# cvg/glue-factory

Hardware: AMD Instinct MI355X
Metric: image-pairs/sec (train step) SP+LightGlue N=2048 d=256 L=9 (higher is better)
Workload: dtype bf16; 1 GPU; configs[1]: SuperPoint + LightGlue train step -- frozen SuperPoint-open forward on 2x32 synthetic 1024x1024 images resident in HBM (view1 = view0 warped by a sampled homography, SURVEY 8(d)(P); first block and the 64-channel 3x3 blocks as fused HIP kernels, library convolutions + fused HIP tails for the 128/256-channel blocks), homography ground truth (gf_gt_nn), LightGlue fwd + loss + bwd + fused; pairs_per_gpu=32, global_batch=32, keypoints=2048, descriptor_dim=256, layers=9, parallelism=dp1

## Files before the change

glue-factory_amd/csrc/assignment.hip:

```cpp
#include <cstdlib>
#include "gf_common.h"
#include "assign_common.h"
#include "gf_amd.h"

#ifndef GF_WRITE_SPLIT
#define GF_WRITE_SPLIT 4
#endif
#ifndef GF_WRITE_ABL
#define GF_WRITE_ABL 0
#endif
#ifndef GF_BWD_SPLIT
#define GF_BWD_SPLIT 4
#endif

namespace {
template <typename T, int D, bool HAS_BIAS>
__global__ __launch_bounds__(256) void rows_lse_kernel(HeadParams p) {
    GF_HEAD_PROLOGUE(T, D)
    float m = GF_NEG_BIG, lsum = 0.f;
    const float* sb = p.sbias ? p.sbias + (int64_t)b * p.Ns : nullptr;
    auto bias = [&](int si, float& v0, float& v1) {
        const float x = sb ? sb[min(si, p.Ns - 1)] * GF_LOG2E : 0.f;
        v0 = si < p.Ns ? x : -INFINITY;
        v1 = 0.f;
    };
    auto body = [&](const T* tile, const float* vec0, const float*, int s0) {
        f32x16 s[2];
        float mx = GF_NEG_BIG;
        const bool plain = !HAS_BIAS && s0 + 64 <= p.Ns;
#pragma unroll
        for (int kb = 0; kb < 2; ++kb) {
#pragma unroll
            for (int r = 0; r < 16; ++r) s[kb][r] = 0.f;
            mma_tile<T, D>(s[kb], tile, kb * 32, of, l31, hi);
            if (plain) {
#pragma unroll
                for (int r = 0; r < 16; ++r) mx = fmaxf(mx, s[kb][r]);
            } else {
#pragma unroll
                for (int g = 0; g < 4; ++g) {
                    f32x4 b4 = *reinterpret_cast<const f32x4*>(vec0 + kb * 32 + 8 * g + 4 * hi);
#pragma unroll
                    for (int e = 0; e < 4; ++e) {
                        float x = s[kb][4 * g + e] * GF_LOG2E + b4[e];
                        s[kb][4 * g + e] = x;
                        mx = fmaxf(mx, x);
                    }
                }
            }
        }
        if (plain) mx *= GF_LOG2E;
        mx = fmaxf(mx, xhalf(mx));
        const float mnew = fmaxf(m, mx);
        float ps = 0.f;
#pragma unroll
        for (int kb = 0; kb < 2; ++kb)
#pragma unroll
            for (int r = 0; r < 16; ++r)
                ps += plain ? fast_exp2(fmaf(s[kb][r], GF_LOG2E, -mnew)) : fast_exp2(s[kb][r] - mnew);
        lsum = lsum * fast_exp2(m - mnew) + ps;
        m = mnew;
    };
    stream_tiles<T, D>(tiles, vecs, othp, 0, p.Ns, p.Ns, bias, body);
    lsum += xhalf(lsum);
    if (orow < p.No && hi == 0) p.f0[(int64_t)b * p.No + orow] = (m + fast_log2(lsum)) * GF_LN2;
}

template <typename T, int D>
__global__ __launch_bounds__(256) void rows_argmax_kernel(HeadParams p) {
    GF_HEAD_PROLOGUE(T, D)
    float best = -INFINITY;
    int bidx = 0x7fffffff;
    const float* sb = p.sbias ? p.sbias + (int64_t)b * p.Ns : nullptr;
    auto bias = [&](int si, float& v0, float& v1) {
        const float x = sb ? sb[min(si, p.Ns - 1)] : 0.f;
        v0 = si < p.Ns ? x : -INFINITY;
        v1 = 0.f;
    };
    auto body = [&](const T* tile, const float* vec0, const float*, int s0) {
        TileArg ta;
        ta.reset();
#pragma unroll
        for (int kb = 0; kb < 2; ++kb) {
            f32x16 s;
#pragma unroll
            for (int r = 0; r < 16; ++r) s[r] = 0.f;
            mma_tile<T, D>(s, tile, kb * 32, of, l31, hi);
#pragma unroll
            for (int g = 0; g < 4; ++g) {
                f32x4 b4 = *reinterpret_cast<const f32x4*>(vec0 + kb * 32 + 8 * g + 4 * hi);
#pragma unroll
                for (int e = 0; e < 4; ++e) {
                    ta.see(p.alpha * s[4 * g + e] + b4[e], kb * 32 + 8 * g + e);
                }
            }
        }
        ta.merge(s0, hi, best, bidx);
    };
    stream_tiles<T, D>(tiles, vecs, othp, 0, p.Ns, p.Ns, bias, body);
    float ob_ = xhalf(best);
    int oi = __shfl_xor(bidx, 32);
    if (ob_ > best || (ob_ == best && oi < bidx)) { best = ob_; bidx = oi; }
    if (orow < p.No && hi == 0) {
        p.f0[(int64_t)b * p.No + orow] = best;
        p.i0[(int64_t)b * p.No + orow] = (bidx == 0x7fffffff) ? 0 : bidx;
    }
}

template <typename T, int D, bool WITH_LSE>
__global__ __launch_bounds__(256, sizeof(T) == 2 ? 2 : 1) void rows_lse_argmax_kernel(HeadParams p) {
    GF_HEAD_PROLOGUE(T, D)
    float m = GF_NEG_BIG, lsum = 0.f;
    float best = -INFINITY;
    int bidx = 0x7fffffff;
    const float* zb = p.g0 + (int64_t)b * p.Ns;
    const float* nb = p.g1 + (int64_t)b * p.Ns;
    auto bias = [&](int si, float& v0, float& v1) {
        const int sc = min(si, p.Ns - 1);
        const float z = zb[sc];
        const float x = fminf(z, 0.f) - log1pf(__expf(-fabsf(z))) - nb[sc];
        v0 = si < p.Ns ? x : -INFINITY;
        v1 = si < p.Ns ? 0.f : -INFINITY;
    };
    auto body = [&](const T* tile, const float* vec0, const float* vec1, int s0) {
        f32x16 s[2];
        float mx = GF_NEG_BIG;
        TileArg ta;
        ta.reset();
#pragma unroll
        for (int kb = 0; kb < 2; ++kb) {
#pragma unroll
            for (int r = 0; r < 16; ++r) s[kb][r] = 0.f;
            mma_tile<T, D>(s[kb], tile, kb * 32, of, l31, hi);
#pragma unroll
            for (int g = 0; g < 4; ++g) {
                f32x4 b4 = *reinterpret_cast<const f32x4*>(vec0 + kb * 32 + 8 * g + 4 * hi);
#pragma unroll
                for (int e = 0; e < 4; ++e) {
                    const float raw = s[kb][4 * g + e];
                    ta.see(p.alpha * raw + b4[e], kb * 32 + 8 * g + e);
                    if (WITH_LSE) mx = fmaxf(mx, raw);
                }
            }
        }
        ta.merge(s0, hi, best, bidx);
        if (WITH_LSE) {
            if (s0 + 64 > p.Ns) {
                mx = GF_NEG_BIG;
#pragma unroll
                for (int kb = 0; kb < 2; ++kb)
#pragma unroll
                    for (int g = 0; g < 4; ++g) {
                        f32x4 v4 = *reinterpret_cast<const f32x4*>(vec1 + kb * 32 + 8 * g + 4 * hi);
#pragma unroll
                        for (int e = 0; e < 4; ++e) {
                            s[kb][4 * g + e] += v4[e];
                            mx = fmaxf(mx, s[kb][4 * g + e]);
                        }
                    }
            }
            mx *= GF_LOG2E;
            mx = fmaxf(mx, xhalf(mx));
            const float mnew = fmaxf(m, mx);
            float ps = 0.f;
#pragma unroll
            for (int kb = 0; kb < 2; ++kb)
#pragma unroll
                for (int r = 0; r < 16; ++r) ps += fast_exp2(fmaf(s[kb][r], GF_LOG2E, -mnew));
            lsum = lsum * fast_exp2(m - mnew) + ps;
            m = mnew;
        }
    };
    stream_tiles<T, D>(tiles, vecs, othp, 0, p.Ns, p.Ns, bias, body);
    float ob_ = xhalf(best);
    int oi = __shfl_xor(bidx, 32);
    if (ob_ > best || (ob_ == best && oi < bidx)) { best = ob_; bidx = oi; }
    if (WITH_LSE) lsum += xhalf(lsum);
    if (orow < p.No && hi == 0) {
        p.f0[(int64_t)b * p.No + orow] = best;
        p.i0[(int64_t)b * p.No + orow] = (bidx == 0x7fffffff) ? 0 : bidx;
        if (WITH_LSE) p.f1[(int64_t)b * p.No + orow] = (m + fast_log2(lsum)) * GF_LN2;
    }
}

template <typename T, int D>
__global__ __launch_bounds__(256) void assign_write_kernel(HeadParams p) {
    GF_HEAD_PROLOGUE(T, D)
#ifdef GF_WRITE_LDPAD
    const int64_t ldo = (p.No + 1 + GF_WRITE_LDPAD - 1) / GF_WRITE_LDPAD * GF_WRITE_LDPAD;
    float* out = reinterpret_cast<float*>(p.out) + (int64_t)b * (p.Ns + 1) * ldo;
#else
    float* out = reinterpret_cast<float*>(p.out) + (int64_t)b * (p.Ns + 1) * (p.No + 1);
    const int64_t ldo = p.No + 1;
#endif
    const float ocb = p.obias ? p.obias[(int64_t)b * p.No + old_] : 0.f;
    const float* sb = p.sbias ? p.sbias + (int64_t)b * p.Ns : nullptr;
    auto bias = [&](int si, float& v0, float& v1) {
        v0 = sb ? sb[min(si, p.Ns - 1)] : 0.f;
        v1 = 0.f;
    };
    float esum = 0.f;
    auto body = [&](const T* tile, const float* vec0, const float*, int s0) {
        TileArg ta;
        ta.reset();
#pragma unroll
        for (int kb = 0; kb < 2; ++kb) {
            f32x16 s;
#pragma unroll
            for (int r = 0; r < 16; ++r) s[r] = 0.f;
            if (!(GF_WRITE_ABL & 1)) mma_tile<T, D>(s, tile, kb * 32, of, l31, hi);
#pragma unroll
            for (int g = 0; g < 4; ++g) {
                f32x4 b4 = *reinterpret_cast<const f32x4*>(vec0 + kb * 32 + 8 * g + 4 * hi);
#pragma unroll
                for (int e = 0; e < 4; ++e) {
                    int si = s0 + kb * 32 + 8 * g + 4 * hi + e;
                    if (si < p.Ns && orow < p.No) {
                        const float v = p.alpha * s[4 * g + e] + b4[e] + ocb;
                        if (!(GF_WRITE_ABL & 2)) out[(int64_t)si * ldo + orow] = v;
                        else if (v == 12345.678f) out[0] = v;
                        if (p.f0 && !(GF_WRITE_ABL & 4)) esum += fast_exp2(v * GF_LOG2E);
                    }
                }
            }
        }
    };
    const int per = ((p.Ns + 63) / 64 + nsp - 1) / nsp * 64;
    const int s_begin = split * per, s_end = min(p.Ns, s_begin + per);
    if (s_begin < s_end) stream_tiles<T, D>(tiles, vecs, othp, s_begin, s_end, p.Ns, bias, body);
    if (split == 0 && orow < p.No && hi == 0) out[(int64_t)p.Ns * ldo + orow] = p.g1 ? p.g1[(int64_t)b * p.No + orow] : 0.f;
    if (ob == 0 && split == 0) {
        for (int si = threadIdx.x; si < p.Ns; si += 256) {
            const float v = p.g0 ? p.g0[(int64_t)b * p.Ns + si] : 0.f;
            out[(int64_t)si * ldo + p.No] = v;
            if (p.f0) esum += fast_exp2(v * GF_LOG2E);
        }
        if (threadIdx.x == 0) out[(int64_t)p.Ns * ldo + p.No] = p.corner;
    }
    if (p.f0) {
        esum = wave_allsum(esum);
        if ((threadIdx.x & 63) == 0) atomicAdd(p.f0 + b, esum);
    }
}

template <typename T, int D>
__global__ __launch_bounds__(256) void dual_softmax_bwd_kernel(HeadParams p) {
    GF_HEAD_PROLOGUE(T, D)
    T* dS = reinterpret_cast<T*>(p.out) + (int64_t)b * p.Ns * p.No;
    const float c2 = p.g1[(int64_t)b * p.No + old_] * GF_LOG2E;
    const float gco = p.g3[(int64_t)b * p.No + old_];
    const float* Gb = p.G ? p.G + (int64_t)b * (p.Ns + 1) * p.ldg : nullptr;
    const int per = ((p.Ns + 63) / 64 + nsp - 1) / nsp * 64;
    const int s_begin = split * per, s_end = min(p.Ns, s_begin + per);
    const float* rb = p.g0 + (int64_t)b * p.Ns;
    const float* grb = p.g2 + (int64_t)b * p.Ns;
    auto bias = [&](int si, float& v0, float& v1) {
        const int sc = min(si, p.Ns - 1);
        const float r_ = rb[sc] * GF_LOG2E, g_ = grb[sc];
        v0 = si < p.Ns ? r_ : INFINITY;
        v1 = si < p.Ns ? g_ : 0.f;
    };
    auto body = [&](const T* tile, const float* vec0, const float* vec1, int s0) {
#pragma unroll
        for (int kb = 0; kb < 2; ++kb) {
            f32x16 s;
#pragma unroll
            for (int r = 0; r < 16; ++r) s[r] = 0.f;
            mma_tile<T, D>(s, tile, kb * 32, of, l31, hi);
#pragma unroll
            for (int g = 0; g < 4; ++g) {
                f32x4 r4 = *reinterpret_cast<const f32x4*>(vec0 + kb * 32 + 8 * g + 4 * hi);
                f32x4 g4 = *reinterpret_cast<const f32x4*>(vec1 + kb * 32 + 8 * g + 4 * hi);
#pragma unroll
                for (int e = 0; e < 4; ++e) {
                    int si = s0 + kb * 32 + 8 * g + 4 * hi + e;
                    if (si < p.Ns && orow < p.No) {
                        float x = s[4 * g + e] * GF_LOG2E;
                        float v = fast_exp2(x - r4[e]) * g4[e] + fast_exp2(x - c2) * gco;
                        if (Gb) v += p.galpha * Gb[(int64_t)si * p.ldg + orow];
                        dS[(int64_t)si * p.No + orow] = from_f32<T>(v);
                    }
                }
            }
        }
    };
    stream_tiles<T, D>(tiles, vecs, othp, s_begin, s_end, p.Ns, bias, body);
}

__global__ void filter_matches_kernel(const float* max0, const int64_t* arg0, const int64_t* arg1, float th,
                                      int64_t* m0, int64_t* m1, float* s0, float* s1, int B, int M, int N) {
    int64_t t = (int64_t)blockIdx.x * blockDim.x + threadIdx.x;
    int64_t tot = (int64_t)B * (M + N);
    if (t >= tot) return;
    int b = t / (M + N);
    int k = t % (M + N);
    const int64_t* a0 = arg0 + (int64_t)b * M;
    const int64_t* a1 = arg1 + (int64_t)b * N;
    if (k < M) {
        int64_t j = a0[k];
        bool mutual = (a1[j] == k);
        float sc = mutual ? __expf(max0[(int64_t)b * M + k]) : 0.f;
        s0[(int64_t)b * M + k] = sc;
        m0[(int64_t)b * M + k] = (mutual && sc > th) ? j : -1;
    } else {
        int j = k - M;
        int64_t i = a1[j];
        bool mutual = (a0[i] == j);
        float sc = mutual ? __expf(max0[(int64_t)b * M + i]) : 0.f;
        s1[(int64_t)b * N + j] = sc;
        m1[(int64_t)b * N + j] = (mutual && sc > th) ? i : -1;
    }
}

enum { K_LSE, K_ARGMAX, K_WRITE, K_BWD, K_LSEARG, K_ZNARG };

template <typename T, int D> int launch_td(int which, const HeadParams& p, hipStream_t st) {
    const int total = ((p.No + 127) / 128) * p.B * (p.nsplit > 1 ? p.nsplit : 1);
    const size_t lds = head_lds<T, D>();
#define GF_LAUNCH(kern)                                             \
    {                                                               \
        if (int e = set_lds(kern<T, D>, lds)) return e;             \
        kern<T, D><<<dim3(total), dim3(256), lds, st>>>(p);         \
        return (int)hipGetLastError();                              \
    }
    switch (which) {
        case K_LSE:
            if (p.sbias) {
                if (int e = set_lds(rows_lse_kernel<T, D, true>, lds)) return e;
                rows_lse_kernel<T, D, true><<<dim3(total), dim3(256), lds, st>>>(p);
            } else {
                if (int e = set_lds(rows_lse_kernel<T, D, false>, lds)) return e;
                rows_lse_kernel<T, D, false><<<dim3(total), dim3(256), lds, st>>>(p);
            }
            return (int)hipGetLastError();
        case K_ARGMAX: GF_LAUNCH(rows_argmax_kernel)
        case K_WRITE: GF_LAUNCH(assign_write_kernel)
        case K_BWD: GF_LAUNCH(dual_softmax_bwd_kernel)
        default: break;
    }
#undef GF_LAUNCH
#define GF_LAUNCH2(flag)                                                              \
    {                                                                                 \
        if (int e = set_lds(rows_lse_argmax_kernel<T, D, flag>, lds)) return e;       \
        rows_lse_argmax_kernel<T, D, flag><<<dim3(total), dim3(256), lds, st>>>(p);   \
        return (int)hipGetLastError();                                                \
    }
    if (which == K_LSEARG) GF_LAUNCH2(true)
    GF_LAUNCH2(false)
#undef GF_LAUNCH2
}

template <typename T> int launch_t(int which, const HeadParams& p, int D, hipStream_t st) {
    switch (D) {
        case 64: return launch_td<T, 64>(which, p, st);
        case 128: return launch_td<T, 128>(which, p, st);
        case 256: return launch_td<T, 256>(which, p, st);
        default: return GF_ERR_UNSUPPORTED;
    }
}

int rejected(const HeadParams& p, int D, int dtype) {
    if (p.B <= 0 || p.No <= 0 || p.Ns <= 0) return GF_ERR_SHAPE;
    if (dtype != GF_F32 && dtype != GF_BF16) return GF_ERR_DTYPE;
    if (D != 64 && D != 128 && D != 256) return GF_ERR_UNSUPPORTED;
    return 0;
}

int launch(int which, const HeadParams& p, int D, int dtype, void* stream) {
    if (p.B <= 0 || p.No <= 0 || p.Ns <= 0) return GF_ERR_SHAPE;
    hipStream_t st = reinterpret_cast<hipStream_t>(stream);
    if (dtype == GF_F32) return launch_t<float>(which, p, D, st);
    if (dtype == GF_BF16) return launch_t<bf16_t>(which, p, D, st);
    return GF_ERR_DTYPE;
}

}

extern "C" int gf_rows_lse(const void* a, const void* b, const float* colbias, float* lse,
                           int B, int M, int N, int D, int dtype, void* stream) {
    HeadParams p = {};
    p.own = a; p.oth = b; p.B = B; p.No = M; p.Ns = N; p.sbias = colbias; p.f0 = lse;
    return launch(K_LSE, p, D, dtype, stream);
}

extern "C" int gf_rows_argmax(const void* a, const void* b, const float* colbias, float alpha,
                              float* rowmax, int64_t* rowarg,
                              int B, int M, int N, int D, int dtype, void* stream) {
    HeadParams p = {};
    p.own = a; p.oth = b; p.B = B; p.No = M; p.Ns = N; p.sbias = colbias; p.alpha = alpha;
    p.f0 = rowmax; p.i0 = rowarg;
    return launch(K_ARGMAX, p, D, dtype, stream);
}

extern "C" int gf_rows_lse_argmax(const void* a, const void* b, const float* bias_z, const float* bias_n,
                                  float alpha, float* lse, float* rowmax, int64_t* rowarg,
                                  int B, int M, int N, int D, int dtype, void* stream) {
    if (bias_z == nullptr || bias_n == nullptr || rowmax == nullptr || rowarg == nullptr) return GF_ERR_SHAPE;
    HeadParams p = {};
    p.own = a; p.oth = b; p.B = B; p.No = M; p.Ns = N; p.g0 = bias_z; p.g1 = bias_n; p.alpha = alpha;
    p.f0 = rowmax; p.i0 = rowarg; p.f1 = lse;
    return launch(lse ? K_LSEARG : K_ZNARG, p, D, dtype, stream);
}

extern "C" int gf_assign_write(const void* a, const void* b, const float* rowbias, const float* colbias,
                               const float* bin_col, const float* bin_row, float alpha, float corner,
                               float* out, float* expsum, int B, int M, int N, int D, int dtype, void* stream) {
    HeadParams p = {};
    p.own = b; p.oth = a; p.B = B; p.No = N; p.Ns = M; p.sbias = rowbias; p.obias = colbias;
    p.alpha = alpha; p.corner = corner; p.g0 = bin_col; p.g1 = bin_row; p.out = out; p.f0 = expsum;
    p.nsplit = GF_WRITE_SPLIT;
    if (int e = rejected(p, D, dtype)) return e;
    if (expsum)
        if (hipError_t e = gf_zero_f32(expsum, (size_t)B, reinterpret_cast<hipStream_t>(stream))) return (int)e;
    return launch(K_WRITE, p, D, dtype, stream);
}

extern "C" int gf_dual_softmax_bwd(const void* a, const void* b, const float* r, const float* c,
                                   const float* gr, const float* gc, const float* G, int64_t ldg,
                                   float galpha, void* dS, int B, int M, int N, int D, int dtype,
                                   void* stream) {
    HeadParams p = {};
    p.own = b; p.oth = a; p.B = B; p.No = N; p.Ns = M;
    p.g0 = r; p.g1 = c; p.g2 = gr; p.g3 = gc; p.G = G; p.ldg = ldg; p.galpha = galpha; p.out = dS;
    p.nsplit = GF_BWD_SPLIT;
    return launch(K_BWD, p, D, dtype, stream);
}

extern "C" int gf_filter_matches(const float* max0, const int64_t* arg0, const int64_t* arg1, float th,
                                 int64_t* m0, int64_t* m1, float* s0, float* s1,
                                 int B, int M, int N, void* stream) {
    if (B <= 0 || M <= 0 || N <= 0) return GF_ERR_SHAPE;
    int64_t tot = (int64_t)B * (M + N);
    int blocks = (int)((tot + 255) / 256);
    filter_matches_kernel<<<dim3(blocks), dim3(256), 0, reinterpret_cast<hipStream_t>(stream)>>>(
        max0, arg0, arg1, th, m0, m1, s0, s1, B, M, N);
    return (int)hipGetLastError();
}
```

Measured before the change: 528.4 image-pairs/s.

## Add ring-buffered MFMA streaming kernels for assignment row LSE/argmax heads

Adds a separate set of bf16 D=256 assignment-head kernels (row log-sum-exp, argmax, and the fused LSE+argmax variants). Each block holds its own rows' descriptors in registers and streams the other side's descriptors through a 2–3 stage LDS ring filled by async 16-byte DMA, with interleaved LDS reads and MFMA. The per-column bias vector is precomputed once into LDS. The aim is to overlap global loads with matrix math and raise MFMA utilisation compared with the generic tiled kernels. It costs extra LDS capacity, which limits Ns to 8192, and adds a second code path that must stay numerically consistent with the original kernels.

```diff
diff --git a/glue-factory_amd/csrc/assign_ring.h b/glue-factory_amd/csrc/assign_ring.h
--- /dev/null
+++ b/glue-factory_amd/csrc/assign_ring.h
@@ -0,0 +1,28 @@
+#pragma once
+#include <hip/hip_runtime.h>
+#include <stdint.h>
+
+namespace gfring {
+
+enum { RING_LSE, RING_ARGMAX, RING_LSEARG, RING_ZNARG };
+
+constexpr int RING_MAX_NS = 8192;
+
+struct RingParams {
+    const void* own;
+    const void* oth;
+    int B, No, Ns;
+    const float* sbias;
+    const float* z;
+    const float* nrm;
+    float alpha;
+    float* f0; float* f1; int64_t* i0;
+};
+
+inline bool applies(const RingParams& p) {
+    return p.Ns <= RING_MAX_NS && (reinterpret_cast<uintptr_t>(p.own) & 15) == 0 && (reinterpret_cast<uintptr_t>(p.oth) & 15) == 0;
+}
+
+int launch(int which, const RingParams& p, hipStream_t st);
+
+}
diff --git a/glue-factory_amd/csrc/assignment.hip b/glue-factory_amd/csrc/assignment.hip
--- a/glue-factory_amd/csrc/assignment.hip
+++ b/glue-factory_amd/csrc/assignment.hip
@@ -1,6 +1,7 @@
 #include <cstdlib>
 #include "gf_common.h"
 #include "assign_common.h"
+#include "assign_ring.h"
 #include "gf_amd.h"
 
 #ifndef GF_WRITE_SPLIT
@@ -314,7 +315,26 @@
 
 enum { K_LSE, K_ARGMAX, K_WRITE, K_BWD, K_LSEARG, K_ZNARG };
 
+int ring_which(int which) {
+    switch (which) {
+        case K_LSE: return gfring::RING_LSE;
+        case K_ARGMAX: return gfring::RING_ARGMAX;
+        case K_LSEARG: return gfring::RING_LSEARG;
+        case K_ZNARG: return gfring::RING_ZNARG;
+        default: return -1;
+    }
+}
+
 template <typename T, int D> int launch_td(int which, const HeadParams& p, hipStream_t st) {
+    if constexpr (sizeof(T) == 2 && D == 256) {
+        const int rw = ring_which(which);
+        if (rw >= 0) {
+            gfring::RingParams rp = {};
+            rp.own = p.own; rp.oth = p.oth; rp.B = p.B; rp.No = p.No; rp.Ns = p.Ns; rp.sbias = p.sbias;
+            rp.z = p.g0; rp.nrm = p.g1; rp.alpha = p.alpha; rp.f0 = p.f0; rp.f1 = p.f1; rp.i0 = p.i0;
+            if (gfring::applies(rp)) return gfring::launch(rw, rp, st);
+        }
+    }
     const int total = ((p.No + 127) / 128) * p.B * (p.nsplit > 1 ? p.nsplit : 1);
     const size_t lds = head_lds<T, D>();
 #define GF_LAUNCH(kern)                                             \
diff --git a/glue-factory_amd/csrc/assignment_ring.hip b/glue-factory_amd/csrc/assignment_ring.hip
--- /dev/null
+++ b/glue-factory_amd/csrc/assignment_ring.hip
@@ -0,0 +1,284 @@
+#include "gf_common.h"
+#include "gf_amd.h"
+#include "attn_common.h"
+#include "assign_common.h"
+#include "assign_ring.h"
+
+#ifndef GF_RING_NW
+#define GF_RING_NW 8
+#endif
+#ifndef GF_RING_NST
+#define GF_RING_NST 3
+#endif
+
+namespace {
+
+using gfattn::FT_TILE;
+using gfattn::as_frag;
+using gfattn::dma16;
+using gfattn::fswz;
+using gfattn::lds_rd128;
+using gfattn::mma16;
+using gfattn::tie;
+using gfattn::wait_lgkm;
+using gfattn::wait_vm;
+using gfring::RingParams;
+
+constexpr int RING_NW = GF_RING_NW, RING_NST = GF_RING_NST;
+constexpr int RING_STAGE = 4 * FT_TILE;
+constexpr int RING_PW = 32 / RING_NW;
+static_assert(RING_NW == 4 || RING_NW == 8, "pieces of a sub-tile divide among 4 or 8 waves");
+static_assert(RING_NST == 2 || RING_NST == 3, "ring depth");
+
+template <typename VecInit, typename Epi>
+__device__ __forceinline__ void ring_stream(const bf16_t* ownrow, const bf16_t* othp, int Ns, VecInit&& vecinit, Epi&& epi) {
+    extern __shared__ __attribute__((aligned(1024))) char smem[];
+    const unsigned lds0 = (unsigned)(size_t)smem;
+    const int lane = threadIdx.x & 63, wave = __builtin_amdgcn_readfirstlane(threadIdx.x >> 6);
+    const int l31 = lane & 31, hi = lane >> 5;
+    const int nt = (Ns + 63) / 64;
+
+    auto issue = [&](int t, int stage) {
+        char* sb = smem + stage * RING_STAGE;
+        const int row0 = min(t, nt - 1) * 64;
+#pragma unroll
+        for (int c = 0; c < 4; ++c)
+#pragma unroll
+            for (int i = 0; i < 8 / RING_NW; ++i) {
+                const int piece = (8 / RING_NW) * wave + i;
+                const int r = piece * 8 + (lane >> 3);
+                const int col = ((lane & 7) ^ fswz(r)) * 8;
+                dma16(othp + (int64_t)min(row0 + r, Ns - 1) * 256 + 64 * c + col, sb + c * FT_TILE + piece * 1024);
+            }
+    };
+#pragma unroll
+    for (int t = 0; t < RING_NST - 1; ++t) issue(t, t);
+
+    bf16x8 of[16];
+#pragma unroll
+    for (int k = 0; k < 16; ++k) of[k] = *reinterpret_cast<const bf16x8*>(ownrow + 16 * k + 8 * hi);
+
+    float* vec = reinterpret_cast<float*>(smem + RING_NST * RING_STAGE);
+    for (int i = threadIdx.x; i < nt * 64; i += RING_NW * 64) vec[i] = i < Ns ? vecinit(i) : -INFINITY;
+    __syncthreads();
+
+    unsigned aR[4];
+    {
+        const unsigned rb = l31 * 128 + 16 * (hi ^ fswz(l31));
+#pragma unroll
+        for (int s = 0; s < 4; ++s) aR[s] = lds0 + (rb ^ (32 * s));
+    }
+    const unsigned aV = lds0 + RING_NST * RING_STAGE + 16 * hi;
+
+    f32x16 sc[2];
+    int stage = 0;
+    for (int t = 0; t < nt; ++t) {
+        wait_vm<(RING_NST - 2) * RING_PW>();
+        __builtin_amdgcn_s_barrier();
+        __builtin_amdgcn_sched_barrier(0);
+        issue(t + RING_NST - 1, stage == 0 ? RING_NST - 1 : stage - 1);
+        unsigned a[4];
+#pragma unroll
+        for (int s = 0; s < 4; ++s) a[s] = aR[s] + stage * RING_STAGE;
+#pragma unroll
+        for (int r = 0; r < 16; ++r) { sc[0][r] = 0.f; sc[1][r] = 0.f; }
+        u32x4 k0[4], k1[4];
+#define GF_AR_RD(dst, J) _Pragma("unroll") for (int s = 0; s < 4; ++s) dst[s] = lds_rd128<((J) & 3) * FT_TILE + ((J) >> 2) * 4096>(a[s]);
+#define GF_AR_MM(src, J) _Pragma("unroll") for (int s = 0; s < 4; ++s) { tie(src[s]); mma16(sc[(J) >> 2], as_frag(src[s]), of[4 * ((J) & 3) + s]); }
+        GF_AR_RD(k0, 0) GF_AR_RD(k1, 1)
+        wait_lgkm<4>(); GF_AR_MM(k0, 0) GF_AR_RD(k0, 2)
+        wait_lgkm<4>(); GF_AR_MM(k1, 1) GF_AR_RD(k1, 3)
+        wait_lgkm<4>(); GF_AR_MM(k0, 2) GF_AR_RD(k0, 4)
+        wait_lgkm<4>(); GF_AR_MM(k1, 3) GF_AR_RD(k1, 5)
+        wait_lgkm<4>(); GF_AR_MM(k0, 4) GF_AR_RD(k0, 6)
+        wait_lgkm<4>(); GF_AR_MM(k1, 5) GF_AR_RD(k1, 7)
+        wait_lgkm<4>(); GF_AR_MM(k0, 6)
+        wait_lgkm<0>(); GF_AR_MM(k1, 7)
+#undef GF_AR_RD
+#undef GF_AR_MM
+        epi(sc, t * 64, aV + t * 256);
+        stage = stage == RING_NST - 1 ? 0 : stage + 1;
+    }
+    wait_vm<0>();
+}
+
+__device__ __forceinline__ void read_rowvec(f32x4 (&b)[2][4], unsigned vaddr) {
+    u32x4 v[8];
+    v[0] = lds_rd128<0>(vaddr);   v[1] = lds_rd128<32>(vaddr);  v[2] = lds_rd128<64>(vaddr);  v[3] = lds_rd128<96>(vaddr);
+    v[4] = lds_rd128<128>(vaddr); v[5] = lds_rd128<160>(vaddr); v[6] = lds_rd128<192>(vaddr); v[7] = lds_rd128<224>(vaddr);
+    wait_lgkm<0>();
+#pragma unroll
+    for (int i = 0; i < 8; ++i) { tie(v[i]); b[i >> 2][i & 3] = __builtin_bit_cast(f32x4, v[i]); }
+}
+
+#define GF_RING_PROLOGUE                                                                          \
+    const int nob = (p.No + 32 * RING_NW - 1) / (32 * RING_NW);                                   \
+    const int lb = xcd_remap(blockIdx.x, nob * p.B);                                              \
+    const int ob = lb % nob, b = lb / nob;                                                        \
+    const int hi = (threadIdx.x & 63) >> 5;                                                       \
+    const int orow = ob * 32 * RING_NW + (threadIdx.x >> 6) * 32 + (threadIdx.x & 31);            \
+    const int old_ = min(orow, p.No - 1);                                                         \
+    const bf16_t* ownrow = reinterpret_cast<const bf16_t*>(p.own) + ((int64_t)b * p.No + old_) * 256; \
+    const bf16_t* othp = reinterpret_cast<const bf16_t*>(p.oth) + (int64_t)b * p.Ns * 256;
+
+template <bool HAS_BIAS>
+__global__ __launch_bounds__(RING_NW * 64, 2) void ring_rows_lse_kernel(RingParams p) {
+    GF_RING_PROLOGUE
+    float m = GF_NEG_BIG, lsum = 0.f;
+    const float* sb = p.sbias ? p.sbias + (int64_t)b * p.Ns : nullptr;
+    auto vecinit = [&](int si) { return sb ? sb[si] * GF_LOG2E : 0.f; };
+    auto epi = [&](f32x16 (&s)[2], int s0, unsigned vaddr) {
+        float mx = GF_NEG_BIG;
+        const bool plain = !HAS_BIAS && s0 + 64 <= p.Ns;
+        if (plain) {
+#pragma unroll
+            for (int kb = 0; kb < 2; ++kb)
+#pragma unroll
+                for (int r = 0; r < 16; ++r) mx = fmaxf(mx, s[kb][r]);
+        } else {
+            f32x4 bv[2][4];
+            read_rowvec(bv, vaddr);
+#pragma unroll
+            for (int kb = 0; kb < 2; ++kb)
+#pragma unroll
+                for (int g = 0; g < 4; ++g)
+#pragma unroll
+                    for (int e = 0; e < 4; ++e) {
+                        float x = s[kb][4 * g + e] * GF_LOG2E + bv[kb][g][e];
+                        s[kb][4 * g + e] = x;
+                        mx = fmaxf(mx, x);
+                    }
+        }
+        if (plain) mx *= GF_LOG2E;
+        mx = fmaxf(mx, xhalf(mx));
+        const float mnew = fmaxf(m, mx);
+        float ps = 0.f;
+#pragma unroll
+        for (int kb = 0; kb < 2; ++kb)
+#pragma unroll
+            for (int r = 0; r < 16; ++r)
+                ps += plain ? fast_exp2(fmaf(s[kb][r], GF_LOG2E, -mnew)) : fast_exp2(s[kb][r] - mnew);
+        lsum = lsum * fast_exp2(m - mnew) + ps;
+        m = mnew;
+    };
+    ring_stream(ownrow, othp, p.Ns, vecinit, epi);
+    lsum += xhalf(lsum);
+    if (orow < p.No && hi == 0) p.f0[(int64_t)b * p.No + orow] = (m + fast_log2(lsum)) * GF_LN2;
+}
+
+__global__ __launch_bounds__(RING_NW * 64, 2) void ring_rows_argmax_kernel(RingParams p) {
+    GF_RING_PROLOGUE
+    float best = -INFINITY;
+    int bidx = 0x7fffffff;
+    const float* sb = p.sbias ? p.sbias + (int64_t)b * p.Ns : nullptr;
+    auto vecinit = [&](int si) { return sb ? sb[si] : 0.f; };
+    auto epi = [&](f32x16 (&s)[2], int s0, unsigned vaddr) {
+        f32x4 bv[2][4];
+        read_rowvec(bv, vaddr);
+        TileArg ta;
+        ta.reset();
+#pragma unroll
+        for (int kb = 0; kb < 2; ++kb)
+#pragma unroll
+            for (int g = 0; g < 4; ++g)
+#pragma unroll
+                for (int e = 0; e < 4; ++e) ta.see(p.alpha * s[kb][4 * g + e] + bv[kb][g][e], kb * 32 + 8 * g + e);
+        ta.merge(s0, hi, best, bidx);
+    };
+    ring_stream(ownrow, othp, p.Ns, vecinit, epi);
+    float ob_ = xhalf(best);
+    int oi = __shfl_xor(bidx, 32);
+    if (ob_ > best || (ob_ == best && oi < bidx)) { best = ob_; bidx = oi; }
+    if (orow < p.No && hi == 0) {
+        p.f0[(int64_t)b * p.No + orow] = best;
+        p.i0[(int64_t)b * p.No + orow] = (bidx == 0x7fffffff) ? 0 : bidx;
+    }
+}
+
+template <bool WITH_LSE>
+__global__ __launch_bounds__(RING_NW * 64, 2) void ring_rows_lse_argmax_kernel(RingParams p) {
+    GF_RING_PROLOGUE
+    float m = GF_NEG_BIG, lsum = 0.f;
+    float best = -INFINITY;
+    int bidx = 0x7fffffff;
+    const float* zb = p.z + (int64_t)b * p.Ns;
+    const float* nb = p.nrm + (int64_t)b * p.Ns;
+    auto vecinit = [&](int si) {
+        const float z = zb[si];
+        return fminf(z, 0.f) - log1pf(__expf(-fabsf(z))) - nb[si];
+    };
+    auto epi = [&](f32x16 (&s)[2], int s0, unsigned vaddr) {
+        f32x4 bv[2][4];
+        read_rowvec(bv, vaddr);
+        float mx = GF_NEG_BIG;
+        TileArg ta;
+        ta.reset();
+#pragma unroll
+        for (int kb = 0; kb < 2; ++kb)
+#pragma unroll
+            for (int g = 0; g < 4; ++g)
+#pragma unroll
+                for (int e = 0; e < 4; ++e) {
+                    const float raw = s[kb][4 * g + e];
+                    ta.see(p.alpha * raw + bv[kb][g][e], kb * 32 + 8 * g + e);
+                    if (WITH_LSE) mx = fmaxf(mx, raw);
+                }
+        ta.merge(s0, hi, best, bidx);
+        if (WITH_LSE) {
+            if (s0 + 64 > p.Ns) {
+                mx = GF_NEG_BIG;
+#pragma unroll
+                for (int kb = 0; kb < 2; ++kb)
+#pragma unroll
+                    for (int g = 0; g < 4; ++g)
+#pragma unroll
+                        for (int e = 0; e < 4; ++e) {
+                            const float v1 = s0 + kb * 32 + 8 * g + 4 * hi + e < p.Ns ? 0.f : -INFINITY;
+                            s[kb][4 * g + e] += v1;
+                            mx = fmaxf(mx, s[kb][4 * g + e]);
+                        }
+            }
+            mx *= GF_LOG2E;
+            mx = fmaxf(mx, xhalf(mx));
+            const float mnew = fmaxf(m, mx);
+            float ps = 0.f;
+#pragma unroll
+            for (int kb = 0; kb < 2; ++kb)
+#pragma unroll
+                for (int r = 0; r < 16; ++r) ps += fast_exp2(fmaf(s[kb][r], GF_LOG2E, -mnew));
+            lsum = lsum * fast_exp2(m - mnew) + ps;
+            m = mnew;
+        }
+    };
+    ring_stream(ownrow, othp, p.Ns, vecinit, epi);
+    float ob_ = xhalf(best);
+    int oi = __shfl_xor(bidx, 32);
+    if (ob_ > best || (ob_ == best && oi < bidx)) { best = ob_; bidx = oi; }
+    if (WITH_LSE) lsum += xhalf(lsum);
+    if (orow < p.No && hi == 0) {
+        p.f0[(int64_t)b * p.No + orow] = best;
+        p.i0[(int64_t)b * p.No + orow] = (bidx == 0x7fffffff) ? 0 : bidx;
+        if (WITH_LSE) p.f1[(int64_t)b * p.No + orow] = (m + fast_log2(lsum)) * GF_LN2;
+    }
+}
+
+template <typename K> int ring_launch(K kern, const RingParams& p, hipStream_t st) {
+    const size_t lds = (size_t)RING_NST * RING_STAGE + (size_t)((p.Ns + 63) / 64) * 64 * sizeof(float);
+    if (int e = gfattn::set_lds(kern, lds)) return e;
+    const int nob = (p.No + 32 * RING_NW - 1) / (32 * RING_NW);
+    kern<<<dim3(nob * p.B), dim3(RING_NW * 64), lds, st>>>(p);
+    return (int)hipGetLastError();
+}
+
+}
+
+int gfring::launch(int which, const RingParams& p, hipStream_t st) {
+    if (!applies(p)) return GF_ERR_UNSUPPORTED;
+    switch (which) {
+        case RING_LSE: return p.sbias ? ring_launch(ring_rows_lse_kernel<true>, p, st) : ring_launch(ring_rows_lse_kernel<false>, p, st);
+        case RING_ARGMAX: return ring_launch(ring_rows_argmax_kernel, p, st);
+        case RING_LSEARG: return ring_launch(ring_rows_lse_argmax_kernel<true>, p, st);
+        case RING_ZNARG: return ring_launch(ring_rows_lse_argmax_kernel<false>, p, st);
+        default: return GF_ERR_UNSUPPORTED;
+    }
+}
```

New measurement: 533.2 image-pairs/s (median of 6 runs). No clear change (+0.9%).
